# BenjSta/bernoulli-var-speech-codec

Measured on AMD Instinct MI355X. Metric: audio-seconds coded per wall-second (encode+decode), 22.05 kHz @ 3 kbit/s, higher is better.
Workload: dtype f32; 1 GPU; BASELINE configs[1]: batch 64 x 5 s utterances per GPU, config_varBitRate @ 3000 bit/s (35 bits/frame), full encode -> BigVGAN decode; one batch at a time on one stream; frames_per_utterance=430, weights=seeded synthetic (checkpoints are LFS pointers), gather=none, streams=1

## Files before the change

bernoulli-var-speech-codec_amd/csrc/k_flow.hip:

```cpp
#include "bvc_internal.h"

namespace bvc {

typedef float f32x4 __attribute__((ext_vector_type(4)));
typedef unsigned u32x4 __attribute__((ext_vector_type(4)));

namespace {

#ifndef BVC_GRU_ROUNDS_FILL
#define BVC_GRU_ROUNDS_FILL 4
#endif
#ifndef BVC_FLOW_EARLYW
#define BVC_FLOW_EARLYW 0
#endif
#ifndef BVC_FLOW_LATEW
#define BVC_FLOW_LATEW 0
#endif
#ifndef BVC_FLOW_STASH
#define BVC_FLOW_STASH 1
#endif
#ifndef BVC_FLOW_PARTNER_WAIT
#define BVC_FLOW_PARTNER_WAIT 1
#endif
#ifndef BVC_FILL_EARLY
#define BVC_FILL_EARLY 0
#endif
#ifndef BVC_GRU_FAST
#define BVC_GRU_FAST 0
#endif
#ifndef BVC_FLOW_PARKV
#define BVC_FLOW_PARKV 2
#endif
#ifndef BVC_FLOW_PARKL
#define BVC_FLOW_PARKL 1
#endif
#ifndef BVC_FLOW_PARK_SET
#define BVC_FLOW_PARK_SET 1
#endif
#ifndef BVC_GRU_FENCE
#define BVC_GRU_FENCE 1
#endif
#ifndef BVC_GRU_DEPTH
#define BVC_GRU_DEPTH 3
#endif
#ifndef BVC_FLOW_POLL_SLEEP
#define BVC_FLOW_POLL_SLEEP 1
#endif
#ifndef BVC_FLOW_DIAG
#define BVC_FLOW_DIAG 0
#endif
constexpr int AUX_SC1 = 16;

__device__ __forceinline__ f32x4 mfma16(float a, float b, f32x4 c) {
    return __builtin_amdgcn_mfma_f32_16x16x4f32(a, b, c, 0, 0, 0);
}
__device__ __forceinline__ float elu1(float v) { return v > 0.0f ? v : expf(v) - 1.0f; }
__device__ __forceinline__ float sigmoid1(float v) { return 1.0f / (1.0f + expf(-v)); }

__device__ __forceinline__ void flow_report(unsigned *status, unsigned code) {
    __hip_atomic_store(status, code, __ATOMIC_RELAXED, __HIP_MEMORY_SCOPE_SYSTEM);
}

struct FlowWg {
    __amdgpu_buffer_rsrc_t rs;
    int lane, wave, mtile, ntile;
    int wmul;
    unsigned spin_limit;
    unsigned *status;
};

#ifndef BVC_FLOW_SPEC
#define BVC_FLOW_SPEC 0
#endif
#ifndef BVC_CHAIN_SPEC
#define BVC_CHAIN_SPEC 0
#endif
#ifndef BVC_CHAIN_G
#define BVC_CHAIN_G 4
#endif
#ifndef BVC_FLOW_MAXCHK
#define BVC_FLOW_MAXCHK 1
#endif
__device__ __forceinline__ unsigned umax3(unsigned a, unsigned b, unsigned c) {
    unsigned r;
    asm("v_max3_u32 %0, %1, %2, %3" : "=v"(r) : "v"(a), "v"(b), "v"(c));
    return r;
}
__device__ __forceinline__ bool is_poison4(const u32x4 v) {
    if (BVC_FLOW_MAXCHK) return umax3(umax3(v[0], v[1], v[2]), v[3], 0u) >= FLOW_POISON;
    return v[0] == FLOW_POISON || v[1] == FLOW_POISON || v[2] == FLOW_POISON || v[3] == FLOW_POISON;
}

struct FlowSrc { unsigned base, vl; };

template <int PER>
__device__ __forceinline__ FlowSrc flow_wait(const FlowWg &g, unsigned buf, int nbdim, int kb0, bool &give_up, unsigned code,
                                             unsigned &spins) {
    FlowSrc s;
    s.base = __builtin_amdgcn_readfirstlane(buf + (unsigned)(g.mtile * nbdim + kb0) * 1024u);
    s.vl = (unsigned)g.lane * 16u;
    const unsigned fl = (unsigned)(g.lane < PER ? g.lane : PER - 1) * 1024u + 63u * 16u + 12u;
    while (!give_up) {
        const unsigned t = __builtin_amdgcn_raw_buffer_load_b32(g.rs, fl, s.base, AUX_SC1);
        if (!__any(t == FLOW_POISON)) break;
        __builtin_amdgcn_s_sleep(BVC_FLOW_POLL_SLEEP);
        if (++spins > g.spin_limit) {
            give_up = true;
            if (g.lane == 0) flow_report(g.status, code);
        }
    }
    return s;
}

#ifndef BVC_FLOW_INORDER
#define BVC_FLOW_INORDER 1
#endif
template <int PER>
__device__ __forceinline__ void flow_issue(const FlowWg &g, const FlowSrc &s, u32x4 (&xr)[PER]) {
#pragma unroll
    for (int u = 0; u < PER; ++u) {
        xr[u] = __builtin_bit_cast(u32x4, __builtin_amdgcn_raw_buffer_load_b128(g.rs, s.vl, s.base + (unsigned)u * 1024u, AUX_SC1));
        if (BVC_FLOW_INORDER) __builtin_amdgcn_sched_barrier(0);
    }
}

typedef const char __attribute__((address_space(1))) *GPtr;
__device__ __forceinline__ GPtr uniform_ptr(const float *w, size_t block) {
    unsigned long long p = reinterpret_cast<unsigned long long>(w) + (block << 10);
    asm volatile("" : "+s"(p));
    return (GPtr)p;
}
__device__ __forceinline__ f32x4 wload(GPtr ub, unsigned lane16, int blk) {
    return *reinterpret_cast<const f32x4 __attribute__((address_space(1))) *>(ub + lane16 + (unsigned)blk * 1024u);
}

typedef u32x4 __attribute__((address_space(3))) *LdsX;
struct SegHook {
    const float *nw; int nwnb; bool pre;
    unsigned long long *st_flags, *st_done;
    LdsX stash;
    const float *fw; size_t fblock; int fstride;
    const float *gw; size_t gblock;
};
constexpr int GRU_EARLY_BLOCKS = 12;
__device__ __forceinline__ SegHook no_hook() { return SegHook{nullptr, 0, false, nullptr, nullptr, (LdsX)0, nullptr, 0, 1, nullptr, 0}; }

template <int PER, int PERN, bool GRUPRE = false, bool FEARLY = false>
__device__ __forceinline__ void lin_segment(const FlowWg &g, const float *w, int wnb, int nb, unsigned buf, bool w_ready,
                                            f32x4 (&wv)[PER], f32x4 &acc, bool &give_up, unsigned code, int kb_off,
                                            const SegHook &hk, f32x4 (&wn)[PERN], f32x4 (&fwv)[PERN], f32x4 (&gqv)[GRU_EARLY_BLOCKS]) {
    const int kb0 = kb_off + g.wave * PER;
    if (PER == 1 && kb0 >= nb) return;
    if (!w_ready) {
        const GPtr ub = uniform_ptr(w, ((size_t)g.ntile * wnb + kb0) * g.wmul);
#pragma unroll
        for (int u = 0; u < PER; ++u) wv[u] = wload(ub, (unsigned)g.lane * 16u, u);
    }
    unsigned spins = 0;
    FlowSrc src;
    if (BVC_FLOW_SPEC) {
        src.base = __builtin_amdgcn_readfirstlane(buf + (unsigned)(g.mtile * nb + kb0) * 1024u);
        src.vl = (unsigned)g.lane * 16u;
    } else {
        src = flow_wait<PER>(g, buf, nb, kb0, give_up, code, spins);
    }
    if (BVC_FLOW_DIAG && hk.st_flags) *hk.st_flags = __builtin_amdgcn_s_memrealtime();
    const f32x4 acc_in = acc;
    u32x4 xr[PER];
    flow_issue<PER>(g, src, xr);
    if (hk.pre) {
        const GPtr ub = uniform_ptr(hk.nw, ((size_t)g.ntile * hk.nwnb + g.wave * PERN) * g.wmul);
#pragma unroll
        for (int u = 0; u < PERN; ++u) wn[u] = wload(ub, (unsigned)g.lane * 16u, u);
    }
    if (GRUPRE) {
        const GPtr ug = uniform_ptr(hk.gw, hk.gblock * g.wmul);
#pragma unroll
        for (int i = 0; i < GRU_EARLY_BLOCKS; ++i) gqv[i] = wload(ug, (unsigned)g.lane * 16u, i);
    }
    if (FEARLY) {
        const GPtr uf = uniform_ptr(hk.fw, hk.fblock * g.wmul);
#pragma unroll
        for (int u = 0; u < PERN; ++u) fwv[u] = hk.fw ? wload(uf, (unsigned)g.lane * 16u, u * hk.fstride) : (f32x4){0.f, 0.f, 0.f, 0.f};
    }
    for (;;) {
        f32x4 a2 = acc_in;
        bool bad = false;
#pragma unroll
        for (int u = 0; u < PER; ++u) {
            if (!BVC_FLOW_INORDER) bad |= is_poison4(xr[u]);
            const f32x4 xv = __builtin_bit_cast(f32x4, xr[u]);
#pragma unroll
            for (int e = 0; e < 4; ++e) a2 = mfma16(wv[u][e], xv[e], a2);
            if (BVC_FLOW_INORDER) __builtin_amdgcn_sched_barrier(0);
        }
        if (BVC_FLOW_INORDER) {
#pragma unroll
            for (int u = 0; u < PER; ++u) bad |= is_poison4(xr[u]);
        }
        if (!(__any(bad) && !give_up)) {
            acc = a2;
            if (BVC_FLOW_STASH && hk.stash) {
#pragma unroll
                for (int u = 0; u < PER; ++u) hk.stash[(kb_off / 8 * PER + u) * 64 + g.lane] = xr[u];
            }
            break;
        }
        if (++spins > g.spin_limit) {
            give_up = true;
            if (g.lane == 0) flow_report(g.status, code);
        }
        flow_issue<PER>(g, src, xr);
    }
    if (BVC_FLOW_DIAG && hk.st_done) *hk.st_done = __builtin_amdgcn_s_memrealtime();
}
template <int PER>
__device__ __forceinline__ void lin_segment(const FlowWg &g, const float *w, int wnb, int nb, unsigned buf, bool w_ready,
                                            f32x4 (&wv)[PER], f32x4 &acc, bool &give_up, unsigned code, int kb_off = 0) {
    f32x4 none[1], nof[1], nog[GRU_EARLY_BLOCKS];
// ... 41 lines not shown
}

template <int PER>
__device__ __forceinline__ void gru_fetch_fresh(const FlowWg &g, unsigned buf, int nb, u32x4 (&xr)[PER], bool &give_up, unsigned code) {
    const int kb0 = g.wave * PER;
    unsigned spins = 0;
    const FlowSrc src = flow_wait<PER>(g, buf, nb, kb0, give_up, code, spins);
    bool again;
    do {
        flow_issue<PER>(g, src, xr);
        bool bad = false;
#pragma unroll
        for (int u = 0; u < PER; ++u) bad |= is_poison4(xr[u]);
        again = __any(bad) && !give_up;
        if (again && ++spins > g.spin_limit) {
            give_up = true;
            if (g.lane == 0) flow_report(g.status, code);
        }
    } while (again);
}

struct FlowFill { const float *w; int wnb; int nb; unsigned buf; };
template <int PER, int GATE>
__device__ __forceinline__ bool fill_active(const FlowWg &g, const FlowFill &f) {
    return GATE != -2 && g.ntile < f.nb && !(PER == 1 && g.wave >= f.nb);
}
template <int PER, int GATE>
__device__ __forceinline__ void fill_issue(const FlowWg &g, const FlowFill &f, f32x4 (&wv)[PER], u32x4 (&xr)[PER]) {
    if (!fill_active<PER, GATE>(g, f)) {
#pragma unroll
        for (int u = 0; u < PER; ++u) { wv[u] = (f32x4){0.f, 0.f, 0.f, 0.f}; xr[u] = (u32x4){0u, 0u, 0u, 0u}; }
        return;
    }
    const int kb0 = g.wave * PER;
    const unsigned l16 = (unsigned)g.lane * 16u;
    const GPtr ub = uniform_ptr(f.w, (GATE >= 0 ? ((size_t)g.ntile * f.wnb + kb0) * 3 + GATE : (size_t)g.ntile * f.wnb + kb0) * g.wmul);
#pragma unroll
    for (int u = 0; u < PER; ++u) wv[u] = wload(ub, l16, GATE >= 0 ? u * 3 : u);
    if (!BVC_FLOW_STASH) gru_issue_known<PER>(g, f.buf, f.nb, xr);
}
template <int PER, int GATE>
__device__ __forceinline__ void fill_multiply(const FlowWg &g, const FlowFill &f, const f32x4 (&wv)[PER], const u32x4 (&xr)[PER], f32x4 &acc,
                                              LdsX stash) {
    if (!fill_active<PER, GATE>(g, f)) return;
    u32x4 xs[PER];
#pragma unroll
    for (int u = 0; u < PER; ++u) xs[u] = BVC_FLOW_STASH ? stash[u * 64 + g.lane] : xr[u];
#pragma unroll
    for (int u = 0; u < PER; ++u) {
        const f32x4 xv = __builtin_bit_cast(f32x4, xs[u]);
#pragma unroll
        for (int e = 0; e < 4; ++e) acc = mfma16(wv[u][e], xv[e], acc);
    }
}

__device__ __forceinline__ u32x4 publishable(f32x4 o, bool rowok) {
    u32x4 b = __builtin_bit_cast(u32x4, o);
#pragma unroll
    for (int j = 0; j < 4; ++j) {
        if (BVC_FLOW_MAXCHK ? b[j] >= FLOW_POISON : b[j] == FLOW_POISON) b[j] = 0x7FC00000u;
        if (!rowok) b[j] = 0u;
    }
    return b;
}

template <bool C, typename A, typename B>
__device__ __forceinline__ decltype(auto) pick(A &a, B &b) {
    if constexpr (C) return (a);
    else return (b);
}

typedef const FlowArgs __attribute__((address_space(4))) *FlowArgsC;

template <typename P>
__device__ __forceinline__ FlowLin L(const P &l) {
    FlowLin r;
    r.w = l.w; r.bias = l.bias; r.wnb = l.wnb; r.pad_ = 0;
    return r;
}

struct FlowCtx {
    FlowWg g;
    FlowArgsC a;
    float *red_lin, *red_gru;
    float *red_chain;
    unsigned sb;
    LdsX stash;
    LdsX gpark;
    LdsX lpark;
    volatile unsigned __attribute__((address_space(3))) *pubflag;
    unsigned par;
    long long t, fr;
    int row;
    bool rowok, give_up;
    bool pre_now;
    bool probe;
    unsigned hopctr;
    f32x4 fgh[3], fgi[3], fd0;
};

__device__ __forceinline__ unsigned long long *flow_stamp_slot(const FlowCtx &c, int hopid, int which) {
    if (!c.probe) return nullptr;
    const auto &a = *c.a;
    return a.probe + ((long long)which * a.T + c.t) * a.probe_nodes + (hopid - a.probe_first);
}
__device__ __forceinline__ void flow_stamp(const FlowCtx &c, int hopid, int which) {
    unsigned long long *p = flow_stamp_slot(c, hopid, which);
    if (p) *p = __builtin_amdgcn_s_memrealtime();
}

template <int EPI, bool ADD, bool REARM_H, int NW>
__device__ __forceinline__ void flow_publish(const FlowCtx &c, int hopid, const float *r, int n0, unsigned ytile, int ntiles, int out,
                                             const f32x4 bias4, const f32x4 add4, const f32x4 mean4, const f32x4 std4, float bitsv,
                                             const f32x4 recv4 = (f32x4){0.f, 0.f, 0.f, 0.f}) {
    const FlowWg &g = c.g;
    const auto &a = *c.a;
    const int lane = g.lane;
    __builtin_amdgcn_s_setprio(3);
    f32x4 v = *reinterpret_cast<const f32x4 *>(r + lane * 4);
#pragma unroll
    for (int w = 1; w < NW; ++w) v += *reinterpret_cast<const f32x4 *>(r + (w * 64 + lane) * 4);
    v += bias4;
    f32x4 o, pr = {0.f, 0.f, 0.f, 0.f};
    if (EPI == FE_ELU || EPI == FE_ELU_KEEP) {
        if (ADD) v += add4;
#pragma unroll
        for (int j = 0; j < 4; ++j) o[j] = elu1(v[j]);
    } else if (EPI == FE_CODE) {
#pragma unroll
        for (int j = 0; j < 4; ++j) {
            pr[j] = sigmoid1(v[j]);
            float z = rintf(pr[j]);
            if (a.var_bit) z = (bitsv > (float)(n0 + j)) ? z : (z != z ? z : 0.5f);
            o[j] = z;
        }
    } else if (EPI == FE_CODE_SEL) {
#pragma unroll
        for (int j = 0; j < 4; ++j) {
            pr[j] = sigmoid1(v[j]);
            float z = rintf(pr[j]);
            z = (bitsv > (float)(n0 + j)) ? z : (z != z ? z : 0.5f);
            o[j] = bitsv < 0.0f ? recv4[j] : z;
        }
    } else {
        if (a.mel && c.rowok) *reinterpret_cast<f32x4 *>(a.mel + c.fr * (ntiles * 16) + n0) = v;
#pragma unroll
        for (int j = 0; j < 4; ++j) o[j] = (v[j] - mean4[j]) / std4[j];
    }
    unsigned pv = FLOW_POISON;
    asm volatile("" : "+v"(pv));
    const u32x4 poison4 = {pv, pv, pv, pv};
    const unsigned ob = (unsigned)(out * 2) * c.sb;
    __builtin_amdgcn_raw_buffer_store_b128(publishable(o, c.rowok), g.rs, ob + c.par * c.sb + ytile, 0, AUX_SC1);
    __builtin_amdgcn_raw_buffer_store_b128(poison4, g.rs, ob + (c.par ^ 1u) * c.sb + ytile, 0, AUX_SC1);
    if (REARM_H) __builtin_amdgcn_raw_buffer_store_b128(poison4, g.rs, (unsigned)(FB_H * 2 + (c.par ^ 1u)) * c.sb + ytile, 0, AUX_SC1);
    if (EPI == FE_ELU_KEEP && c.rowok && a.keep) *reinterpret_cast<f32x4 *>(a.keep + c.fr * (ntiles * 16) + n0) = o;
    if ((EPI == FE_CODE || EPI == FE_CODE_SEL) && c.rowok) {
        *reinterpret_cast<f32x4 *>(a.codes + c.fr * (ntiles * 16) + n0) = o;
        if (a.prob) *reinterpret_cast<f32x4 *>(a.prob + c.fr * (ntiles * 16) + n0) = pr;
    }
    __builtin_amdgcn_s_setprio(0);
    flow_stamp(c, hopid, 1);
}

template <int PER, int EPI, bool TWO, bool ADD, bool PRE_IN, bool PRE_OUT, int PERN, bool REARM_H = false, int FGATE = -2, int NW = 8, bool GRUPRE = false>
__device__ __forceinline__ void flow_layer(FlowCtx &c, int hopid, const FlowLin l0, int src0, const FlowLin l1, int src1,
                                           int nb, int ntiles, int out, f32x4 (&wv)[PER], const FlowLin nxt, f32x4 (&wn)[PERN],
                                           f32x4 (&gq)[GRU_EARLY_BLOCKS],
                                           const f32x4 acc0 = (f32x4){0.f, 0.f, 0.f, 0.f}, const FlowFill fill = FlowFill{nullptr, 0, 0, 0u},
                                           f32x4 *facc = nullptr) {
    const FlowWg &g = c.g;
    const auto &a = *c.a;
    f32x4 fw[PERN];
    u32x4 fx[PERN];
    if (g.ntile >= ntiles) {
        if (PRE_OUT && c.pre_now) {
#pragma unroll
            for (int u = 0; u < PERN; ++u) wn[u] = (f32x4){0.f, 0.f, 0.f, 0.f};
        }
        if (FGATE != -2) {
            fill_issue<PERN, FGATE>(g, fill, fw, fx);
            fill_multiply<PERN, FGATE>(g, fill, fw, fx, *facc, c.stash);
        }
        if (BVC_GRU_FAST && GRUPRE) {
#pragma unroll
            for (int i = 0; i < GRU_EARLY_BLOCKS; ++i) gq[i] = (f32x4){0.f, 0.f, 0.f, 0.f};
        }
        return;
    }
    int lane = g.lane;
    const int wave = g.wave;
    asm volatile("" : "+v"(lane));
    const unsigned code = (unsigned)((c.t << 4) | (unsigned)hopid) | 0x80000000u;
    const int n0 = g.ntile * 16 + (lane >> 4) * 4;
    const unsigned ytile = (unsigned)((g.mtile * ntiles + g.ntile) * 1024 + lane * 16);
    flow_stamp(c, hopid, 0);
    f32x4 bias4 = {0.f, 0.f, 0.f, 0.f}, add4 = {0.f, 0.f, 0.f, 0.f}, mean4 = {0.f, 0.f, 0.f, 0.f}, std4 = {1.f, 1.f, 1.f, 1.f};
    float bitsv = 0.0f;
    f32x4 recv4 = {0.f, 0.f, 0.f, 0.f};
    if (wave == 0) {
        if (l0.bias) bias4 = *reinterpret_cast<const f32x4 *>(l0.bias + n0);
        if (ADD && c.rowok) add4 = *reinterpret_cast<const f32x4 *>(a.part0 + c.fr * (ntiles * 16) + n0);
        if (EPI == FE_CODE && a.var_bit && c.rowok) bitsv = a.bits[c.fr];
        if (EPI == FE_CODE_SEL && c.rowok) {
            bitsv = a.bits[c.fr];
            recv4 = *reinterpret_cast<const f32x4 *>(a.codes_in + c.fr * (ntiles * 16) + n0);
        }
        if (EPI == FE_MEL) {
            mean4 = *reinterpret_cast<const f32x4 *>(a.mean + n0);
            std4 = *reinterpret_cast<const f32x4 *>(a.stdv + n0);
        }
    }
    f32x4 acc = acc0;
    constexpr bool EARLY = BVC_FLOW_EARLYW && PRE_OUT && PER > 1;
    constexpr bool FEARLY = BVC_FILL_EARLY && FGATE != -2 && PER > 1;
    SegHook hk = no_hook();
    if (BVC_FLOW_DIAG) { hk.st_flags = flow_stamp_slot(c, hopid, 2); hk.st_done = flow_stamp_slot(c, hopid, 3); }
    if (BVC_FLOW_STASH && FGATE == 0) hk.stash = c.stash;
    if (PER == 1) {
        for (int off = 0; off < nb; off += NW)
            lin_segment<PER, PERN>(g, l0.w, l0.wnb, nb, (unsigned)(src0 * 2 + c.par) * c.sb, false, wv, acc, c.give_up, code, off, hk, wn, fw, gq);
        if (TWO)
            for (int off = 0; off < nb; off += NW)
                lin_segment<PER, PERN>(g, l1.w, l1.wnb, nb, (unsigned)(src1 * 2 + c.par) * c.sb, false, wv, acc, c.give_up, code, off, hk, wn, fw, gq);
    } else {
        SegHook hl = hk;
        if (EARLY) { hl.nw = nxt.w; hl.nwnb = nxt.wnb; hl.pre = c.pre_now; }
        constexpr bool GP = BVC_GRU_FAST && GRUPRE;
        if (GP) { hl.gw = a.w_ihx; hl.gblock = ((size_t)g.ntile * 2 * a.hb + wave * PER) * 3; }
        if (FEARLY && fill_active<PERN, FGATE>(g, fill)) {
            static_assert(!FEARLY || BVC_FLOW_STASH, "BVC_FILL_EARLY requests the quantum's weights only: its input must come from the stash");
            hl.fw = fill.w;
            hl.fblock = FGATE >= 0 ? ((size_t)g.ntile * fill.wnb + wave * PERN) * 3 + FGATE : (size_t)g.ntile * fill.wnb + wave * PERN;
            hl.fstride = FGATE >= 0 ? 3 : 1;
        }
        if (TWO) {
            lin_segment<PER>(g, l0.w, l0.wnb, nb, (unsigned)(src0 * 2 + c.par) * c.sb, PRE_IN, wv, acc, c.give_up, code);
            lin_segment<PER, PERN, GP, FEARLY>(g, l1.w, l1.wnb, nb, (unsigned)(src1 * 2 + c.par) * c.sb, false, wv, acc, c.give_up, code, 0, hl, wn, fw, gq);
        } else {
            lin_segment<PER, PERN, GP, FEARLY>(g, l0.w, l0.wnb, nb, (unsigned)(src0 * 2 + c.par) * c.sb, PRE_IN, wv, acc, c.give_up, code, 0, hl, wn, fw, gq);
        }
    }
    constexpr bool LATE = BVC_FLOW_LATEW && PRE_OUT && !EARLY;
    if (PRE_OUT && !EARLY && !LATE && c.pre_now) {
        const GPtr ub = uniform_ptr(nxt.w, ((size_t)g.ntile * nxt.wnb + wave * PERN) * g.wmul);
#pragma unroll
        for (int u = 0; u < PERN; ++u) wn[u] = wload(ub, (unsigned)lane * 16u, u);
    }
    if (FGATE != -2 && !FEARLY) fill_issue<PERN, FGATE>(g, fill, fw, fx);
    float *r = c.red_lin + (c.hopctr & 1u) * (NW * 256);
    ++c.hopctr;
    *reinterpret_cast<f32x4 *>(r + (wave * 64 + lane) * 4) = acc;
    __syncthreads();
    if (BVC_FLOW_DIAG) flow_stamp(c, hopid, 4);
    if (LATE && wave != 0 && c.pre_now) {
        const GPtr ub = uniform_ptr(nxt.w, ((size_t)g.ntile * nxt.wnb + wave * PERN) * g.wmul);
#pragma unroll
        for (int u = 0; u < PERN; ++u) wn[u] = wload(ub, (unsigned)lane * 16u, u);
    }
    if (wave == 0) {
        if constexpr (EPI == FE_CODE_SEL) flow_publish<EPI, ADD, REARM_H, NW>(c, hopid, r, n0, ytile, ntiles, out, bias4, add4, mean4, std4, bitsv, recv4);
        else flow_publish<EPI, ADD, REARM_H, NW>(c, hopid, r, n0, ytile, ntiles, out, bias4, add4, mean4, std4, bitsv);
        if (BVC_FLOW_PARTNER_WAIT && NW == 8 && FGATE != -2) *c.pubflag = c.hopctr;
        if (LATE && c.pre_now) {
            const GPtr ub = uniform_ptr(nxt.w, ((size_t)g.ntile * nxt.wnb + wave * PERN) * g.wmul);
#pragma unroll
            for (int u = 0; u < PERN; ++u) wn[u] = wload(ub, (unsigned)lane * 16u, u);
        }
    } else if (BVC_FLOW_PARTNER_WAIT && NW == 8 && wave == 4 && FGATE != -2) {
        for (int i = 0; i < 4096 && *c.pubflag != c.hopctr; ++i) __builtin_amdgcn_s_sleep(2);
    }
    if (FGATE != -2) fill_multiply<PERN, FGATE>(g, fill, fw, fx, *facc, c.stash);
    if (BVC_FLOW_DIAG) flow_stamp(c, hopid, 5);
}

template <int PER, int EPI, bool ADD, bool PRE_IN, bool PRE_OUT, int PERN, bool REARM_H, int NW, bool TWO = false>
__device__ __forceinline__ void flow_layer_chains(FlowCtx &c, int hopid, const FlowLin l0, int src0, int nb, int ntiles, int out,
                                                  f32x4 (&wv)[PER], const FlowLin nxt, f32x4 (&wn)[PERN], int mt0, int nch, long long T,
                                                  const FlowLin lfirst = FlowLin{nullptr, nullptr, 0, 0}, int srcfirst = 0) {
    static_assert(PER > 1, "narrow inputs take the per-chain path");
    static_assert(NW == 8, "two sets of four publishing waves");
    constexpr int GM = 4;
    const int G = nch >= 3 ? BVC_CHAIN_G : 1;
    FlowWg &g = c.g;
    const auto &a = *c.a;
    if (g.ntile >= ntiles) {
        if (PRE_OUT) {
#pragma unroll
            for (int u = 0; u < PERN; ++u) wn[u] = (f32x4){0.f, 0.f, 0.f, 0.f};
        }
        return;
    }
    int lane = g.lane;
    const int wave = g.wave;
    asm volatile("" : "+v"(lane));
    const unsigned code = (unsigned)((c.t << 4) | (unsigned)hopid) | 0x80000000u;
    const int n0 = g.ntile * 16 + (lane >> 4) * 4;
    const int kb0 = wave * PER;
    const unsigned bufb = (unsigned)(src0 * 2 + c.par) * c.sb;
    if (!PRE_IN) {
        const GPtr ub = uniform_ptr(l0.w, ((size_t)g.ntile * l0.wnb + kb0) * g.wmul);
#pragma unroll
        for (int u = 0; u < PER; ++u) wv[u] = wload(ub, (unsigned)lane * 16u, u);
    }
    f32x4 bias4 = {0.f, 0.f, 0.f, 0.f}, mean4 = {0.f, 0.f, 0.f, 0.f}, std4 = {1.f, 1.f, 1.f, 1.f};
    if (l0.bias) bias4 = *reinterpret_cast<const f32x4 *>(l0.bias + n0);
    if (EPI == FE_MEL) {
        mean4 = *reinterpret_cast<const f32x4 *>(a.mean + n0);
        std4 = *reinterpret_cast<const f32x4 *>(a.stdv + n0);
    }
    unsigned spins = 0;
    flow_stamp(c, hopid, 0);
    f32x4 wfirst[TWO ? PER : 1];
    if (TWO) {
        const GPtr ub = uniform_ptr(lfirst.w, ((size_t)g.ntile * lfirst.wnb + kb0) * g.wmul);
#pragma unroll
        for (int u = 0; u < PER; ++u) wfirst[u] = wload(ub, (unsigned)lane * 16u, u);
    }
    u32x4 xc[PER], xn[PER];
    for (int g0 = 0, grp = 0; g0 < nch; g0 += G, ++grp) {
        const int gn = nch - g0 < G ? nch - g0 : G;
        f32x4 accs[GM];
#pragma unroll
        for (int k = 0; k < GM; ++k) accs[k] = (f32x4){0.f, 0.f, 0.f, 0.f};
#pragma unroll
// ... 312 lines not shown

#ifndef BVC_FLOW_WAVES_PER_SIMD
#define BVC_FLOW_WAVES_PER_SIMD 2
#endif
#define FLOW_EACH_CHAIN(...)                                                                                            \
    for (int ci_ = 0; ci_ < nch; ++ci_) {                                                                               \
        c.g.mtile = mt0 + ci_;                                                                                          \
        c.row = c.g.mtile * 16 + (c.g.lane & 15);                                                                       \
        c.rowok = c.row < a.B;                                                                                          \
        c.fr = (long long)c.row * T + t;                                                                                \
        c.pre_now = ci_ == nch - 1;                                                                                     \
        __VA_ARGS__;                                                                                                    \
    }

template <int PERH, bool ENCODE, bool FILL, int NW = 8, bool MULTI = false, int FOLD = -1, bool CONCEAL = false>
__global__ __launch_bounds__(NW * 64, NW == 8 ? BVC_FLOW_WAVES_PER_SIMD : 1) void bvrnn_flow_kernel(const FlowArgs *a0) {
    static_assert(!(MULTI && FILL), "the filler quanta are per chain: not built for interleaved chains");
    static_assert(!CONCEAL || ENCODE, "the concealing decoder is a variant of the encode program");
    constexpr int EPI3 = CONCEAL ? FE_CODE_SEL : FE_CODE;
    extern __shared__ __attribute__((aligned(16))) float lds[];
    const int tid = threadIdx.x;
    FlowCtx c;
    FlowArgsC ap = (FlowArgsC)(unsigned long long)a0;
    c.a = ap;
    c.red_lin = lds;
    c.red_gru = lds + 2 * NW * 256;
    c.red_chain = lds + 2 * NW * 256 + NW * 6 * 256;
    c.stash = (LdsX)(lds + 2 * NW * 256) + (tid >> 6) * (PERH * 64);
    c.gpark = (LdsX)(lds + 2 * NW * 256 + NW * 8 * 256) + (tid >> 6) * (6 * 64);
    c.lpark = (LdsX)(lds + 2 * NW * 256 + NW * 8 * 256) + (tid >> 6) * (8 * 64);
    static_assert(!(BVC_FLOW_PARKL && BVC_GRU_FAST), "one use of the parking region");
    c.pubflag = (volatile unsigned __attribute__((address_space(3))) *)(lds + 2 * NW * 256 + NW * 8 * 256 + NW * 8 * 256);
    if (FILL && tid == 0) c.pubflag[0] = 0xFFFFFFFFu;
    c.g.lane = tid & 63;
    c.g.wave = __builtin_amdgcn_readfirstlane(tid >> 6);
    const int bid = blockIdx.x, xcd = bid & 7, slot = bid >> 3;
    const int MT = ap->MT;
    const int MG = MULTI ? ap->MG : 1;
    const int MTG = MULTI ? (MT + MG - 1) / MG : MT;
    c.g.ntile = (slot / MTG) * 8 + xcd;
    const int mt0 = (slot % MTG) * MG;
    const int nch = MULTI ? (MT - mt0 < MG ? MT - mt0 : MG) : 1;
    c.g.mtile = mt0;
    if (ap->dbg_withhold && bid == 0) return;
    if (c.g.ntile >= ap->NTG) return;
    c.g.rs = __builtin_amdgcn_make_buffer_rsrc(ap->flow, 0, (int)(FB_COUNT * 2u * ap->slot_bytes), 0x00020000);
    c.sb = ap->slot_bytes;
    c.g.spin_limit = ap->spin_limit;
    c.g.wmul = ap->dbg_hot_w ? 0 : 1;
    c.g.status = ap->status;
    c.row = c.g.mtile * 16 + (c.g.lane & 15);
    c.rowok = c.row < ap->B;
    c.give_up = false;
    c.pre_now = true;
    c.probe = ap->probe != nullptr && bid == ap->probe_wg && tid == ap->probe_wave * 64;
    c.hopctr = 0;
    const int hb = ap->hb, zb = ap->zb, xb = ap->xb;
    const long long T = ap->T;
    const bool hfull = c.g.ntile < hb;
    f32x4 wa[PERH], wb[PERH], w1[1];
    f32x4 gq[GRU_EARLY_BLOCKS];
    constexpr bool GFAST = FILL && PERH == 8 && BVC_GRU_FAST && !MULTI;
    constexpr bool GPRE = GFAST;
    if (GFAST && hfull) {
        const GPtr ux = uniform_ptr(ap->w_ihx, (((size_t)c.g.ntile * 2 * hb + c.g.wave * PERH) * 3 + 12) * c.g.wmul);
#pragma unroll
        for (int i = 0; i < 6; ++i) c.gpark[i * 64 + c.g.lane] = __builtin_bit_cast(u32x4, wload(ux, (unsigned)c.g.lane * 16u, i));
    }
    constexpr bool PK = BVC_FLOW_PARKV && FILL && !MULTI;
    constexpr bool PL = BVC_FLOW_PARKL && FILL && !MULTI && PERH == 8;
    constexpr bool P8 = PK && BVC_FLOW_PARK_SET == 1, P9 = PK && (BVC_FLOW_PARK_SET == 1 || (!ENCODE && BVC_FLOW_PARKV >= 2)),
                   P12 = PK && BVC_FLOW_PARK_SET == 0, P13 = PK && (BVC_FLOW_PARK_SET == 0 || (!ENCODE && BVC_FLOW_PARKV >= 2));
    f32x4 k8[P8 ? PERH : 1], k9[P9 ? PERH : 1], k12[P12 ? PERH : 1], k13[P13 ? PERH : 1];
    {
        auto park = [&](auto &k, const FlowLin l) {
            const GPtr u = uniform_ptr(l.w, hfull ? (size_t)c.g.ntile * l.wnb + c.g.wave * PERH : 0);
#pragma unroll
            for (int i = 0; i < PERH; ++i) k[i] = wload(u, (unsigned)c.g.lane * 16u, i);
        };
        if constexpr (P8) park(k8, L(ap->dec1));
        if constexpr (P9) park(k9, L(ap->dec2));
        if constexpr (P12) park(k12, L(ap->px1));
        if constexpr (P13) park(k13, L(ap->px2));
    }
    {
        const FlowLin first = ENCODE ? L(ap->enc0h) : L(ap->dec0h);
        const GPtr ub = uniform_ptr(first.w, hfull ? (size_t)c.g.ntile * first.wnb + c.g.wave * PERH : 0);
#pragma unroll
        for (int u = 0; u < PERH; ++u) wa[u] = wload(ub, (unsigned)c.g.lane * 16u, u);
        if constexpr (PL) {
#pragma unroll
            for (int u = 0; u < PERH; ++u) c.lpark[u * 64 + c.g.lane] = __builtin_bit_cast(u32x4, wa[u]);
        }
    }
    for (long long t = 0; t < T; ++t) {
        if constexpr (PL) {
#pragma unroll
            for (int u = 0; u < PERH; ++u) wa[u] = __builtin_bit_cast(f32x4, c.lpark[u * 64 + c.g.lane]);
        }
        asm volatile("" : "+s"(ap));
        c.a = ap;
        const auto &a = *ap;
        c.t = t;
        c.par = (unsigned)(t & 1);
        c.fr = (long long)c.row * T + t;
        const f32x4 zero4 = {0.f, 0.f, 0.f, 0.f};
        if (FILL) {
#pragma unroll
            for (int q = 0; q < 3; ++q) { c.fgh[q] = zero4; c.fgi[q] = zero4; }
            c.fd0 = zero4;
        }
        const unsigned hsrc = (unsigned)(FB_H * 2 + c.par) * c.sb, zsrc = (unsigned)(FB_Q3 * 2 + c.par) * c.sb;
        constexpr int G0 = FILL ? 0 : -2, G1 = FILL ? 1 : -2, G2 = FILL ? 2 : -2, GP = FILL ? -1 : -2;
        const FlowFill f_hh = {a.w_hh, hb, hb, hsrc}, f_d0 = {a.dec0h.w, a.dec0h.wnb, hb, hsrc}, f_iz = {a.w_ihz, 2 * hb, hb, zsrc};
        const bool folded = FOLD < 0 ? a.pxc.w != nullptr : FOLD == 1;
        if constexpr (!MULTI) {
            auto &w8 = pick<P8>(k8, wb);  auto &w9 = pick<P9>(k9, wa);  auto &w12 = pick<P12>(k12, wa);  auto &w13 = pick<P13>(k13, wb);
            if (ENCODE) {
                flow_layer<PERH, FE_ELU, false, !CONCEAL, true, true, PERH, false, G0, NW>(c, 1, L(a.enc0h), FB_H, L(a.enc0h), 0, hb, hb, FB_E1, wa, L(a.enc1), wb, gq, zero4, f_hh, &c.fgh[0]);
                flow_layer<PERH, FE_ELU, false, false, true, false, PERH, true, G1, NW>(c, 2, L(a.enc1), FB_E1, L(a.enc1), 0, hb, hb, FB_E2, wb, L(a.enc1), wa, gq, zero4, f_hh, &c.fgh[1]);
                flow_layer<PERH, EPI3, false, false, false, false, PERH, false, G2, NW>(c, 3, L(a.enc2), FB_E2, L(a.enc2), 0, hb, zb, FB_ZC, wa, L(a.enc2), wb, gq, zero4, f_hh, &c.fgh[2]);
                flow_layer<1, FE_ELU, false, false, false, true, PERH, false, GP, NW>(c, 4, L(a.pz0), FB_ZC, L(a.pz0), 0, zb, hb, FB_Q1, w1, L(a.pz1), wa, gq, zero4, f_d0, &c.fd0);
                flow_layer<PERH, FE_ELU, false, false, true, true, PERH, false, -2, NW>(c, 5, L(a.pz1), FB_Q1, L(a.pz1), 0, hb, hb, FB_Q2, wa, L(a.pz2), wb, gq);
                if (FILL) {
                    FlowLin d0 = L(a.dec0z);
                    d0.bias = a.dec0h.bias;
                    flow_layer<PERH, FE_ELU, false, false, true, true, PERH, false, -2, NW>(c, 6, L(a.pz2), FB_Q2, L(a.pz2), 0, hb, hb, FB_Q3, wb, d0, wa, gq);
                    flow_layer<PERH, FE_ELU, false, false, true, !P8, PERH, false, G0, NW>(c, 7, d0, FB_Q3, d0, 0, hb, hb, FB_D1, wa, L(a.dec1), wb, gq, c.fd0, f_iz, &c.fgi[0]);
                } else {
                    flow_layer<PERH, FE_ELU, false, false, true, true, PERH, false, -2, NW>(c, 6, L(a.pz2), FB_Q2, L(a.pz2), 0, hb, hb, FB_Q3, wb, L(a.dec0h), wa, gq);
                    flow_layer<PERH, FE_ELU, true, false, true, true, PERH, false, -2, NW>(c, 7, L(a.dec0h), FB_H, L(a.dec0z), FB_Q3, hb, hb, FB_D1, wa, L(a.dec1), wb, gq);
                }
                flow_layer<PERH, FE_ELU, false, false, true, !P9, PERH, false, G1, NW>(c, 8, L(a.dec1), FB_D1, L(a.dec1), 0, hb, hb, FB_D2, w8, L(a.dec2), wa, gq, zero4, f_iz, &c.fgi[1]);
                if (folded) {
                    flow_layer<PERH, FE_ELU_KEEP, false, false, true, true, PERH, false, G2, NW>(c, 9, L(a.dec2), FB_D2, L(a.dec2), 0, hb, hb, FB_D3, w9, L(a.pxc), wb, gq, zero4, f_iz, &c.fgi[2]);
                    flow_layer<PERH, FE_ELU, false, false, true, !P12, PERH, false, -2, NW>(c, 11, L(a.pxc), FB_D3, L(a.pxc), 0, hb, hb, FB_G1, wb, L(a.px1), wa, gq);
                } else {
                    flow_layer<PERH, FE_ELU, false, false, true, false, PERH, false, G2, NW>(c, 9, L(a.dec2), FB_D2, L(a.dec2), 0, hb, hb, FB_D3, w9, L(a.dec2), wb, gq, zero4, f_iz, &c.fgi[2]);
                    flow_layer<PERH, FE_MEL, false, false, false, false, PERH, false, -2, NW>(c, 10, L(a.dec3), FB_D3, L(a.dec3), 0, hb, xb, FB_DN, wa, L(a.dec3), wb, gq);
                }
            } else {
                flow_layer<PERH, FE_ELU, false, true, true, !P8, PERH, false, G0, NW>(c, 7, L(a.dec0h), FB_H, L(a.dec0h), 0, hb, hb, FB_D1, wa, L(a.dec1), wb, gq, zero4, f_hh, &c.fgh[0]);
                flow_layer<PERH, FE_ELU, false, false, true, !P9, PERH, true, G1, NW>(c, 8, L(a.dec1), FB_D1, L(a.dec1), 0, hb, hb, FB_D2, w8, L(a.dec2), wa, gq, zero4, f_hh, &c.fgh[1]);
                if (folded) {
                    flow_layer<PERH, FE_ELU_KEEP, false, false, true, true, PERH, false, G2, NW>(c, 9, L(a.dec2), FB_D2, L(a.dec2), 0, hb, hb, FB_D3, w9, L(a.pxc), wb, gq, zero4, f_hh, &c.fgh[2]);
                    flow_layer<PERH, FE_ELU, false, false, true, !P12, PERH, false, -2, NW>(c, 11, L(a.pxc), FB_D3, L(a.pxc), 0, hb, hb, FB_G1, wb, L(a.px1), wa, gq);
                } else {
                    flow_layer<PERH, FE_ELU, false, false, true, false, PERH, false, G2, NW>(c, 9, L(a.dec2), FB_D2, L(a.dec2), 0, hb, hb, FB_D3, w9, L(a.dec2), wb, gq, zero4, f_hh, &c.fgh[2]);
                    flow_layer<PERH, FE_MEL, false, false, false, false, PERH, false, -2, NW>(c, 10, L(a.dec3), FB_D3, L(a.dec3), 0, hb, xb, FB_DN, wa, L(a.dec3), wb, gq);
                }
            }
            if (!folded)
                flow_layer<1, FE_ELU, false, false, false, !P12, PERH, false, -2, NW>(c, 11, L(a.px0), FB_DN, L(a.px0), 0, xb, hb, FB_G1, w1, L(a.px1), wa, gq);
            flow_layer<PERH, FE_ELU, false, false, true, !P13, PERH, false, -2, NW>(c, 12, L(a.px1), FB_G1, L(a.px1), 0, hb, hb, FB_G2, w12, L(a.px2), wb, gq);
            flow_layer<PERH, FE_ELU, false, false, true, false, PERH, false, -2, NW, GPRE>(c, 13, L(a.px2), FB_G2, L(a.px2), 0, hb, hb, FB_G3, w13, L(a.px2), wa, gq);
            flow_gru<PERH, ENCODE, PERH, FILL, NW>(c, 14, hb, ENCODE ? L(a.enc0h) : L(a.dec0h), wa, gq);
        } else {
            constexpr bool E = ENCODE;
            if (E) {
                flow_layer_chains<PERH, FE_ELU, !CONCEAL, true, true, PERH, false, NW>(c, 1, L(a.enc0h), FB_H, hb, hb, FB_E1, wa, L(a.enc1), wb, mt0, nch, T);
                flow_layer_chains<PERH, FE_ELU, false, true, false, PERH, true, NW>(c, 2, L(a.enc1), FB_E1, hb, hb, FB_E2, wb, L(a.enc1), wa, mt0, nch, T);
                flow_layer_chains<PERH, EPI3, false, false, false, PERH, false, NW>(c, 3, L(a.enc2), FB_E2, hb, zb, FB_ZC, wa, L(a.enc2), wb, mt0, nch, T);
                FLOW_EACH_CHAIN(flow_layer<1, FE_ELU, false, false, false, true, PERH, false, -2, NW>(c, 4, L(a.pz0), FB_ZC, L(a.pz0), 0, zb, hb, FB_Q1, w1, L(a.pz1), wa, gq));
                flow_layer_chains<PERH, FE_ELU, false, true, true, PERH, false, NW>(c, 5, L(a.pz1), FB_Q1, hb, hb, FB_Q2, wa, L(a.pz2), wb, mt0, nch, T);
                flow_layer_chains<PERH, FE_ELU, false, true, false, PERH, false, NW>(c, 6, L(a.pz2), FB_Q2, hb, hb, FB_Q3, wb, L(a.pz2), wa, mt0, nch, T);
                {
                    const GPtr ub = uniform_ptr(a.dec0z.w, ((size_t)c.g.ntile * a.dec0z.wnb + c.g.wave * PERH) * c.g.wmul);
#pragma unroll
                    for (int u = 0; u < PERH; ++u) wa[u] = wload(ub, (unsigned)c.g.lane * 16u, u);
                    FlowLin d0 = L(a.dec0z);
                    d0.bias = a.dec0h.bias;
                    flow_layer_chains<PERH, FE_ELU, false, true, true, PERH, false, NW, true>(c, 7, d0, FB_Q3, hb, hb, FB_D1, wa, L(a.dec1), wb, mt0, nch, T, L(a.dec0h), FB_H);
                }
                flow_layer_chains<PERH, FE_ELU, false, true, true, PERH, false, NW>(c, 8, L(a.dec1), FB_D1, hb, hb, FB_D2, wb, L(a.dec2), wa, mt0, nch, T);
                if (folded) {
                    flow_layer_chains<PERH, FE_ELU_KEEP, false, true, true, PERH, false, NW>(c, 9, L(a.dec2), FB_D2, hb, hb, FB_D3, wa, L(a.pxc), wb, mt0, nch, T);
                    flow_layer_chains<PERH, FE_ELU, false, true, true, PERH, false, NW>(c, 11, L(a.pxc), FB_D3, hb, hb, FB_G1, wb, L(a.px1), wa, mt0, nch, T);
                } else {
                    flow_layer_chains<PERH, FE_ELU, false, true, false, PERH, false, NW>(c, 9, L(a.dec2), FB_D2, hb, hb, FB_D3, wa, L(a.dec2), wb, mt0, nch, T);
                }
            } else {
                flow_layer_chains<PERH, FE_ELU, true, true, true, PERH, false, NW>(c, 7, L(a.dec0h), FB_H, hb, hb, FB_D1, wa, L(a.dec1), wb, mt0, nch, T);
                flow_layer_chains<PERH, FE_ELU, false, true, true, PERH, true, NW>(c, 8, L(a.dec1), FB_D1, hb, hb, FB_D2, wb, L(a.dec2), wa, mt0, nch, T);
                if (folded) {
                    flow_layer_chains<PERH, FE_ELU_KEEP, false, true, true, PERH, false, NW>(c, 9, L(a.dec2), FB_D2, hb, hb, FB_D3, wa, L(a.pxc), wb, mt0, nch, T);
                    flow_layer_chains<PERH, FE_ELU, false, true, true, PERH, false, NW>(c, 11, L(a.pxc), FB_D3, hb, hb, FB_G1, wb, L(a.px1), wa, mt0, nch, T);
                } else {
                    flow_layer_chains<PERH, FE_ELU, false, true, false, PERH, false, NW>(c, 9, L(a.dec2), FB_D2, hb, hb, FB_D3, wa, L(a.dec2), wb, mt0, nch, T);
                }
            }
            if (!folded) {
                flow_layer_chains<PERH, FE_MEL, false, false, false, PERH, false, NW>(c, 10, L(a.dec3), FB_D3, hb, xb, FB_DN, wa, L(a.dec3), wb, mt0, nch, T);
                FLOW_EACH_CHAIN(flow_layer<1, FE_ELU, false, false, false, true, PERH, false, -2, NW>(c, 11, L(a.px0), FB_DN, L(a.px0), 0, xb, hb, FB_G1, w1, L(a.px1), wa, gq));
            }
            flow_layer_chains<PERH, FE_ELU, false, true, true, PERH, false, NW>(c, 12, L(a.px1), FB_G1, hb, hb, FB_G2, wa, L(a.px2), wb, mt0, nch, T);
            flow_layer_chains<PERH, FE_ELU, false, true, false, PERH, false, NW>(c, 13, L(a.px2), FB_G2, hb, hb, FB_G3, wb, L(a.px2), wa, mt0, nch, T);
            flow_gru_chains<PERH, ENCODE, PERH, NW>(c, 14, hb, ENCODE ? L(a.enc0h) : L(a.dec0h), wa, mt0, nch, T);
        }
// ... 159 lines not shown
```

Measured before the change: 7069 audio-seconds/s.

## Poll next layer's readiness flags inside GRU fill multiply to overlap wait

Adds a fill_multiply_poll path that interleaves polling of the next hop's poison flags with the fill-gate MFMA work, slicing the multiply so flag loads are hidden behind compute. When readiness is observed during the fill, the next lin_segment skips its own spin-wait via a FlowSeen record. It also prefetches the next layer's weights before the fill for the enc2 hop (W3 flag). This aims to cut inter-layer synchronization latency in the persistent recurrent flow kernel. It adds scheduling barriers, extra state, and more polling traffic, and it could raise register pressure.

```diff
diff --git a/bernoulli-var-speech-codec_amd/csrc/k_flow.hip b/bernoulli-var-speech-codec_amd/csrc/k_flow.hip
--- a/bernoulli-var-speech-codec_amd/csrc/k_flow.hip
+++ b/bernoulli-var-speech-codec_amd/csrc/k_flow.hip
@@ -48,6 +48,18 @@
 #endif
 #ifndef BVC_FLOW_DIAG
 #define BVC_FLOW_DIAG 0
+#endif
+#ifndef BVC_FILL_POLL
+#define BVC_FILL_POLL 1
+#endif
+#ifndef BVC_FILL_POLL_SLICE
+#define BVC_FILL_POLL_SLICE 8
+#endif
+#ifndef BVC_FILL_POLL_FIRST
+#define BVC_FILL_POLL_FIRST 0
+#endif
+#ifndef BVC_FILL_POLL_WAVES
+#define BVC_FILL_POLL_WAVES 0
 #endif
 constexpr int AUX_SC1 = 16;
 
@@ -92,14 +104,24 @@
 }
 
 struct FlowSrc { unsigned base, vl; };
-
+struct FlowSeen { bool seen; unsigned spins; };
+
+template <int PER>
+__device__ __forceinline__ FlowSrc flow_src(const FlowWg &g, unsigned buf, int nbdim, int kb0) {
+    FlowSrc s;
+    s.base = __builtin_amdgcn_readfirstlane(buf + (unsigned)(g.mtile * nbdim + kb0) * 1024u);
+    s.vl = (unsigned)g.lane * 16u;
+    return s;
+}
+template <int PER>
+__device__ __forceinline__ unsigned flow_flag_offset(const FlowWg &g) {
+    return (unsigned)(g.lane < PER ? g.lane : PER - 1) * 1024u + 63u * 16u + 12u;
+}
 template <int PER>
 __device__ __forceinline__ FlowSrc flow_wait(const FlowWg &g, unsigned buf, int nbdim, int kb0, bool &give_up, unsigned code,
                                              unsigned &spins) {
-    FlowSrc s;
-    s.base = __builtin_amdgcn_readfirstlane(buf + (unsigned)(g.mtile * nbdim + kb0) * 1024u);
-    s.vl = (unsigned)g.lane * 16u;
-    const unsigned fl = (unsigned)(g.lane < PER ? g.lane : PER - 1) * 1024u + 63u * 16u + 12u;
+    const FlowSrc s = flow_src<PER>(g, buf, nbdim, kb0);
+    const unsigned fl = flow_flag_offset<PER>(g);
     while (!give_up) {
         const unsigned t = __builtin_amdgcn_raw_buffer_load_b32(g.rs, fl, s.base, AUX_SC1);
         if (!__any(t == FLOW_POISON)) break;
@@ -148,7 +170,8 @@
 template <int PER, int PERN, bool GRUPRE = false, bool FEARLY = false>
 __device__ __forceinline__ void lin_segment(const FlowWg &g, const float *w, int wnb, int nb, unsigned buf, bool w_ready,
                                             f32x4 (&wv)[PER], f32x4 &acc, bool &give_up, unsigned code, int kb_off,
-                                            const SegHook &hk, f32x4 (&wn)[PERN], f32x4 (&fwv)[PERN], f32x4 (&gqv)[GRU_EARLY_BLOCKS]) {
+                                            const SegHook &hk, f32x4 (&wn)[PERN], f32x4 (&fwv)[PERN], f32x4 (&gqv)[GRU_EARLY_BLOCKS],
+                                            FlowSeen *pre = nullptr) {
     const int kb0 = kb_off + g.wave * PER;
     if (PER == 1 && kb0 >= nb) return;
     if (!w_ready) {
@@ -158,13 +181,19 @@
     }
     unsigned spins = 0;
     FlowSrc src;
+    bool preseen = false;
     if (BVC_FLOW_SPEC) {
         src.base = __builtin_amdgcn_readfirstlane(buf + (unsigned)(g.mtile * nb + kb0) * 1024u);
         src.vl = (unsigned)g.lane * 16u;
+    } else if (pre && pre->seen) {
+        src = flow_src<PER>(g, buf, nb, kb0);
+        spins = pre->spins;
+        pre->seen = false;
+        preseen = true;
     } else {
         src = flow_wait<PER>(g, buf, nb, kb0, give_up, code, spins);
     }
-    if (BVC_FLOW_DIAG && hk.st_flags) *hk.st_flags = __builtin_amdgcn_s_memrealtime();
+    if (BVC_FLOW_DIAG && hk.st_flags && !preseen) *hk.st_flags = __builtin_amdgcn_s_memrealtime();
     const f32x4 acc_in = acc;
     u32x4 xr[PER];
     flow_issue<PER>(g, src, xr);
@@ -312,6 +341,63 @@
 #pragma unroll
         for (int e = 0; e < 4; ++e) acc = mfma16(wv[u][e], xv[e], acc);
     }
+}
+
+struct FlowNext { int src, hop, nb, ntiles; const float *w; int wnb; };
+__device__ __forceinline__ FlowNext no_next() { return FlowNext{-1, 0, 0, 0, nullptr, 0}; }
+template <int PER, int GATE>
+__device__ __forceinline__ void fill_multiply_poll(const FlowWg &g, const f32x4 (&wv)[PER], const u32x4 (&xr)[PER], f32x4 &acc, LdsX stash,
+                                                   unsigned nbuf, int nnb, bool &give_up, unsigned code, FlowSeen &out,
+                                                   unsigned long long *st_flags) {
+    static_assert(BVC_FILL_POLL_SLICE % 4 == 0 && BVC_FILL_POLL_SLICE >= 4 && (PER * 4) % BVC_FILL_POLL_SLICE == 0, "a slice is a whole number of k-blocks");
+    constexpr int SB = BVC_FILL_POLL_SLICE / 4;
+    constexpr int LB = SB < 2 ? SB : 2;
+    u32x4 xs[PER];
+#pragma unroll
+    for (int u = 0; u < LB; ++u) xs[u] = BVC_FLOW_STASH ? stash[u * 64 + g.lane] : xr[u];
+    const unsigned base = flow_src<PER>(g, nbuf, nnb, g.wave * PER).base;
+    const unsigned fl = flow_flag_offset<PER>(g);
+    unsigned spins = 0, t = 0u;
+    unsigned seen = __builtin_amdgcn_readfirstlane((unsigned)give_up), poll = 0u;
+    f32x4 a2 = acc;
+#pragma unroll
+    for (int u0 = 0; u0 < PER; u0 += LB) {
+        if (u0 % SB == 0) {
+            poll = (!seen && u0 * 4 >= BVC_FILL_POLL_FIRST) ? 1u : 0u;
+            if (poll) t = __builtin_amdgcn_raw_buffer_load_b32(g.rs, fl, base, AUX_SC1);
+        }
+#pragma unroll
+        for (int u = u0 + LB; u < u0 + 2 * LB && u < PER; ++u) xs[u] = BVC_FLOW_STASH ? stash[u * 64 + g.lane] : xr[u];
+        __builtin_amdgcn_sched_barrier(0);
+#pragma unroll
+        for (int u = u0; u < u0 + LB; ++u) {
+            const f32x4 xv = __builtin_bit_cast(f32x4, xs[u]);
+#pragma unroll
+            for (int e = 0; e < 4; ++e) a2 = mfma16(wv[u][e], xv[e], a2);
+        }
+        __builtin_amdgcn_sched_barrier(0);
+        if ((u0 + LB) % SB == 0 && poll) {
+            asm volatile("" : "+v"(t));
+            if (__builtin_amdgcn_readfirstlane((unsigned)!__any(t == FLOW_POISON))) {
+                seen = 1u;
+                if (BVC_FLOW_DIAG && st_flags) *st_flags = __builtin_amdgcn_s_memrealtime();
+            } else {
+                if (u0 + LB >= PER) __builtin_amdgcn_s_sleep(BVC_FLOW_POLL_SLEEP);
+                if (++spins > g.spin_limit) {
+                    give_up = true;
+                    seen = 1u;
+                    if (g.lane == 0) flow_report(g.status, code);
+                }
+            }
+        }
+    }
+    acc = a2;
+    if (!seen) {
+        flow_wait<PER>(g, nbuf, nnb, g.wave * PER, give_up, code, spins);
+        if (BVC_FLOW_DIAG && st_flags) *st_flags = __builtin_amdgcn_s_memrealtime();
+    }
+    out.seen = true;
+    out.spins = spins;
 }
 
 __device__ __forceinline__ u32x4 publishable(f32x4 o, bool rowok) {
@@ -355,6 +441,7 @@
     bool rowok, give_up;
     bool pre_now;
     bool probe;
+    FlowSeen nseen;
     unsigned hopctr;
     f32x4 fgh[3], fgi[3], fd0;
 };
@@ -428,7 +515,7 @@
                                            int nb, int ntiles, int out, f32x4 (&wv)[PER], const FlowLin nxt, f32x4 (&wn)[PERN],
                                            f32x4 (&gq)[GRU_EARLY_BLOCKS],
                                            const f32x4 acc0 = (f32x4){0.f, 0.f, 0.f, 0.f}, const FlowFill fill = FlowFill{nullptr, 0, 0, 0u},
-                                           f32x4 *facc = nullptr) {
+                                           f32x4 *facc = nullptr, const FlowNext nx = no_next()) {
     const FlowWg &g = c.g;
     const auto &a = *c.a;
     f32x4 fw[PERN];
@@ -498,7 +585,7 @@
             lin_segment<PER>(g, l0.w, l0.wnb, nb, (unsigned)(src0 * 2 + c.par) * c.sb, PRE_IN, wv, acc, c.give_up, code);
             lin_segment<PER, PERN, GP, FEARLY>(g, l1.w, l1.wnb, nb, (unsigned)(src1 * 2 + c.par) * c.sb, false, wv, acc, c.give_up, code, 0, hl, wn, fw, gq);
         } else {
-            lin_segment<PER, PERN, GP, FEARLY>(g, l0.w, l0.wnb, nb, (unsigned)(src0 * 2 + c.par) * c.sb, PRE_IN, wv, acc, c.give_up, code, 0, hl, wn, fw, gq);
+            lin_segment<PER, PERN, GP, FEARLY>(g, l0.w, l0.wnb, nb, (unsigned)(src0 * 2 + c.par) * c.sb, PRE_IN, wv, acc, c.give_up, code, 0, hl, wn, fw, gq, &c.nseen);
         }
     }
     constexpr bool LATE = BVC_FLOW_LATEW && PRE_OUT && !EARLY;
@@ -530,7 +617,23 @@
     } else if (BVC_FLOW_PARTNER_WAIT && NW == 8 && wave == 4 && FGATE != -2) {
         for (int i = 0; i < 4096 && *c.pubflag != c.hopctr; ++i) __builtin_amdgcn_s_sleep(2);
     }
-    if (FGATE != -2) fill_multiply<PERN, FGATE>(g, fill, fw, fx, *facc, c.stash);
+    if constexpr (BVC_FILL_POLL && FGATE != -2 && PERN == 8) {
+        const bool nown = nx.src >= 0 && g.ntile < nx.ntiles && fill_active<PERN, FGATE>(g, fill);
+        if (nown && nx.w) {
+            const GPtr ub = uniform_ptr(nx.w, ((size_t)g.ntile * nx.wnb + wave * PERN) * g.wmul);
+#pragma unroll
+            for (int u = 0; u < PERN; ++u) wn[u] = wload(ub, (unsigned)lane * 16u, u);
+            __builtin_amdgcn_sched_barrier(0);
+        }
+        if (nown && (!BVC_FILL_POLL_WAVES || (wave & 3) == 0)) {
+            fill_multiply_poll<PERN, FGATE>(g, fw, fx, *facc, c.stash, (unsigned)(nx.src * 2 + c.par) * c.sb, nx.nb, c.give_up,
+                                            (unsigned)((c.t << 4) | (unsigned)nx.hop) | 0x80000000u, c.nseen, BVC_FLOW_DIAG ? flow_stamp_slot(c, nx.hop, 2) : nullptr);
+        } else {
+            fill_multiply<PERN, FGATE>(g, fill, fw, fx, *facc, c.stash);
+        }
+    } else if (FGATE != -2) {
+        fill_multiply<PERN, FGATE>(g, fill, fw, fx, *facc, c.stash);
+    }
     if (BVC_FLOW_DIAG) flow_stamp(c, hopid, 5);
 }
 
@@ -949,6 +1052,7 @@
     c.row = c.g.mtile * 16 + (c.g.lane & 15);
     c.rowok = c.row < ap->B;
     c.give_up = false;
+    c.nseen = FlowSeen{false, 0u};
     c.pre_now = true;
     c.probe = ap->probe != nullptr && bid == ap->probe_wg && tid == ap->probe_wave * 64;
     c.hopctr = 0;
@@ -1012,35 +1116,37 @@
         const FlowFill f_hh = {a.w_hh, hb, hb, hsrc}, f_d0 = {a.dec0h.w, a.dec0h.wnb, hb, hsrc}, f_iz = {a.w_ihz, 2 * hb, hb, zsrc};
         const bool folded = FOLD < 0 ? a.pxc.w != nullptr : FOLD == 1;
         if constexpr (!MULTI) {
+            const FlowNext n8 = {FB_D1, 8, hb, hb, nullptr, 0}, n9 = {FB_D2, 9, hb, hb, nullptr, 0}, n11 = {FB_D3, 11, hb, hb, nullptr, 0};
+            constexpr bool W3 = BVC_FILL_POLL != 0 && FILL && PERH == 8;
             auto &w8 = pick<P8>(k8, wb);  auto &w9 = pick<P9>(k9, wa);  auto &w12 = pick<P12>(k12, wa);  auto &w13 = pick<P13>(k13, wb);
             if (ENCODE) {
-                flow_layer<PERH, FE_ELU, false, !CONCEAL, true, true, PERH, false, G0, NW>(c, 1, L(a.enc0h), FB_H, L(a.enc0h), 0, hb, hb, FB_E1, wa, L(a.enc1), wb, gq, zero4, f_hh, &c.fgh[0]);
-                flow_layer<PERH, FE_ELU, false, false, true, false, PERH, true, G1, NW>(c, 2, L(a.enc1), FB_E1, L(a.enc1), 0, hb, hb, FB_E2, wb, L(a.enc1), wa, gq, zero4, f_hh, &c.fgh[1]);
-                flow_layer<PERH, EPI3, false, false, false, false, PERH, false, G2, NW>(c, 3, L(a.enc2), FB_E2, L(a.enc2), 0, hb, zb, FB_ZC, wa, L(a.enc2), wb, gq, zero4, f_hh, &c.fgh[2]);
-                flow_layer<1, FE_ELU, false, false, false, true, PERH, false, GP, NW>(c, 4, L(a.pz0), FB_ZC, L(a.pz0), 0, zb, hb, FB_Q1, w1, L(a.pz1), wa, gq, zero4, f_d0, &c.fd0);
+                flow_layer<PERH, FE_ELU, false, !CONCEAL, true, true, PERH, false, G0, NW>(c, 1, L(a.enc0h), FB_H, L(a.enc0h), 0, hb, hb, FB_E1, wa, L(a.enc1), wb, gq, zero4, f_hh, &c.fgh[0], FlowNext{FB_E1, 2, hb, hb, nullptr, 0});
+                flow_layer<PERH, FE_ELU, false, false, true, false, PERH, true, G1, NW>(c, 2, L(a.enc1), FB_E1, L(a.enc1), 0, hb, hb, FB_E2, wb, L(a.enc1), wa, gq, zero4, f_hh, &c.fgh[1], FlowNext{FB_E2, 3, hb, zb, a.enc2.w, a.enc2.wnb});
+                flow_layer<PERH, EPI3, false, false, W3, false, PERH, false, G2, NW>(c, 3, L(a.enc2), FB_E2, L(a.enc2), 0, hb, zb, FB_ZC, wa, L(a.enc2), wb, gq, zero4, f_hh, &c.fgh[2]);
+                flow_layer<1, FE_ELU, false, false, false, true, PERH, false, GP, NW>(c, 4, L(a.pz0), FB_ZC, L(a.pz0), 0, zb, hb, FB_Q1, w1, L(a.pz1), wa, gq, zero4, f_d0, &c.fd0, FlowNext{FB_Q1, 5, hb, hb, nullptr, 0});
                 flow_layer<PERH, FE_ELU, false, false, true, true, PERH, false, -2, NW>(c, 5, L(a.pz1), FB_Q1, L(a.pz1), 0, hb, hb, FB_Q2, wa, L(a.pz2), wb, gq);
                 if (FILL) {
                     FlowLin d0 = L(a.dec0z);
                     d0.bias = a.dec0h.bias;
                     flow_layer<PERH, FE_ELU, false, false, true, true, PERH, false, -2, NW>(c, 6, L(a.pz2), FB_Q2, L(a.pz2), 0, hb, hb, FB_Q3, wb, d0, wa, gq);
-                    flow_layer<PERH, FE_ELU, false, false, true, !P8, PERH, false, G0, NW>(c, 7, d0, FB_Q3, d0, 0, hb, hb, FB_D1, wa, L(a.dec1), wb, gq, c.fd0, f_iz, &c.fgi[0]);
+                    flow_layer<PERH, FE_ELU, false, false, true, !P8, PERH, false, G0, NW>(c, 7, d0, FB_Q3, d0, 0, hb, hb, FB_D1, wa, L(a.dec1), wb, gq, c.fd0, f_iz, &c.fgi[0], n8);
                 } else {
                     flow_layer<PERH, FE_ELU, false, false, true, true, PERH, false, -2, NW>(c, 6, L(a.pz2), FB_Q2, L(a.pz2), 0, hb, hb, FB_Q3, wb, L(a.dec0h), wa, gq);
                     flow_layer<PERH, FE_ELU, true, false, true, true, PERH, false, -2, NW>(c, 7, L(a.dec0h), FB_H, L(a.dec0z), FB_Q3, hb, hb, FB_D1, wa, L(a.dec1), wb, gq);
                 }
-                flow_layer<PERH, FE_ELU, false, false, true, !P9, PERH, false, G1, NW>(c, 8, L(a.dec1), FB_D1, L(a.dec1), 0, hb, hb, FB_D2, w8, L(a.dec2), wa, gq, zero4, f_iz, &c.fgi[1]);
+                flow_layer<PERH, FE_ELU, false, false, true, !P9, PERH, false, G1, NW>(c, 8, L(a.dec1), FB_D1, L(a.dec1), 0, hb, hb, FB_D2, w8, L(a.dec2), wa, gq, zero4, f_iz, &c.fgi[1], n9);
                 if (folded) {
-                    flow_layer<PERH, FE_ELU_KEEP, false, false, true, true, PERH, false, G2, NW>(c, 9, L(a.dec2), FB_D2, L(a.dec2), 0, hb, hb, FB_D3, w9, L(a.pxc), wb, gq, zero4, f_iz, &c.fgi[2]);
+                    flow_layer<PERH, FE_ELU_KEEP, false, false, true, true, PERH, false, G2, NW>(c, 9, L(a.dec2), FB_D2, L(a.dec2), 0, hb, hb, FB_D3, w9, L(a.pxc), wb, gq, zero4, f_iz, &c.fgi[2], n11);
                     flow_layer<PERH, FE_ELU, false, false, true, !P12, PERH, false, -2, NW>(c, 11, L(a.pxc), FB_D3, L(a.pxc), 0, hb, hb, FB_G1, wb, L(a.px1), wa, gq);
                 } else {
                     flow_layer<PERH, FE_ELU, false, false, true, false, PERH, false, G2, NW>(c, 9, L(a.dec2), FB_D2, L(a.dec2), 0, hb, hb, FB_D3, w9, L(a.dec2), wb, gq, zero4, f_iz, &c.fgi[2]);
                     flow_layer<PERH, FE_MEL, false, false, false, false, PERH, false, -2, NW>(c, 10, L(a.dec3), FB_D3, L(a.dec3), 0, hb, xb, FB_DN, wa, L(a.dec3), wb, gq);
                 }
             } else {
-                flow_layer<PERH, FE_ELU, false, true, true, !P8, PERH, false, G0, NW>(c, 7, L(a.dec0h), FB_H, L(a.dec0h), 0, hb, hb, FB_D1, wa, L(a.dec1), wb, gq, zero4, f_hh, &c.fgh[0]);
-                flow_layer<PERH, FE_ELU, false, false, true, !P9, PERH, true, G1, NW>(c, 8, L(a.dec1), FB_D1, L(a.dec1), 0, hb, hb, FB_D2, w8, L(a.dec2), wa, gq, zero4, f_hh, &c.fgh[1]);
+                flow_layer<PERH, FE_ELU, false, true, true, !P8, PERH, false, G0, NW>(c, 7, L(a.dec0h), FB_H, L(a.dec0h), 0, hb, hb, FB_D1, wa, L(a.dec1), wb, gq, zero4, f_hh, &c.fgh[0], n8);
+                flow_layer<PERH, FE_ELU, false, false, true, !P9, PERH, true, G1, NW>(c, 8, L(a.dec1), FB_D1, L(a.dec1), 0, hb, hb, FB_D2, w8, L(a.dec2), wa, gq, zero4, f_hh, &c.fgh[1], n9);
                 if (folded) {
-                    flow_layer<PERH, FE_ELU_KEEP, false, false, true, true, PERH, false, G2, NW>(c, 9, L(a.dec2), FB_D2, L(a.dec2), 0, hb, hb, FB_D3, w9, L(a.pxc), wb, gq, zero4, f_hh, &c.fgh[2]);
+                    flow_layer<PERH, FE_ELU_KEEP, false, false, true, true, PERH, false, G2, NW>(c, 9, L(a.dec2), FB_D2, L(a.dec2), 0, hb, hb, FB_D3, w9, L(a.pxc), wb, gq, zero4, f_hh, &c.fgh[2], n11);
                     flow_layer<PERH, FE_ELU, false, false, true, !P12, PERH, false, -2, NW>(c, 11, L(a.pxc), FB_D3, L(a.pxc), 0, hb, hb, FB_G1, wb, L(a.px1), wa, gq);
                 } else {
                     flow_layer<PERH, FE_ELU, false, false, true, false, PERH, false, G2, NW>(c, 9, L(a.dec2), FB_D2, L(a.dec2), 0, hb, hb, FB_D3, w9, L(a.dec2), wb, gq, zero4, f_hh, &c.fgh[2]);
```

Result: slower. 6643 audio-seconds/s (-6.0%).
